# fabrii4/AutoEncoder-FFT

Measured on AMD Instinct MI355X. Metric: frames/s fwd+bwd (FFT mode, 512x512, 4 layers), higher is better.
Workload: dtype f32; 1 GPU; cfg3-P2: 512x512x3 frames, 4 pairs 3->8->16->32->64, 5x5, pool 2/layer, FFT mode, fwd + 1 loop-body iteration per pair (operator form); every step produces reconstructions, batch-mean gradients, updated weights and the per-pair post-update MSE partial sums -- the sums themselves are formed by the next step's gradient launch (no per-step MSE read-back inside the timed loop); frames_per_gpu=32, global_batch=32, parallelism=dp1

## Files before the change

### autoencoder-fft_amd/csrc/fft_kernels.hip

```cpp
#include "internal.h"
#include "device_util.h"
#include "fft_common.h"
#include <hip/hip_ext.h>
#include <math.h>
#include <map>
#include <mutex>
#include <vector>

namespace aefft {

__device__ float2 g_tw[TW_N];

hipError_t upload_twiddles(hipStream_t st)
{
    static std::vector<float2> host;
    if (host.empty()) {
        host.resize(TW_N);
        for (int k = 0; k < TW_N; ++k) {
            double a = -2.0 * M_PI * (double)k / (double)TW_N;
            host[k] = make_float2((float)cos(a), (float)sin(a));
        }
    }
    hipError_t e = hipMemcpyToSymbolAsync(HIP_SYMBOL(g_tw), host.data(), sizeof(float2) * TW_N, 0, hipMemcpyHostToDevice, st);
    if (e != hipSuccess) return e;
    return hipStreamSynchronize(st);
}

const float2* twiddle_table()
{
    void* p = nullptr;
    if (hipGetSymbolAddress(&p, HIP_SYMBOL(g_tw)) != hipSuccess) return nullptr;
    return static_cast<const float2*>(p);
}

bool fft_size_supported(int n) { return n >= 8 && n <= 2048 && (n & (n - 1)) == 0; }

template <int DIR> __device__ __forceinline__ float2 twid(int idx)
{
    float2 w = g_tw[idx];
    if (DIR > 0) w.y = -w.y;
    return w;
}

template <int N> __device__ __forceinline__ void pass_sync()
{
    if constexpr (N / 8 <= 64) __builtin_amdgcn_wave_barrier();
    else __syncthreads();
}

template <int N, int R, int S, int DIR>
__device__ __forceinline__ void fft_pass(float2* s, int t, float2 w1)
{
    constexpr int T = N / 8;
    constexpr int E = 8 / R;
    constexpr int n = N / S;
    float2 a[8];
#pragma unroll
    for (int v = 0; v < E; ++v) {
        const int ib = t + T * v;
#pragma unroll
        for (int tt = 0; tt < R; ++tt) a[v * R + tt] = s[pad_idx(ib + tt * (N / R))];
    }
    pass_sync<N>();
#pragma unroll
    for (int v = 0; v < E; ++v) {
        const int ib = t + T * v;
        const int p = ib / S, q = ib % S;
        Dft<R, DIR>::run(&a[v * R]);
        if constexpr (n > R) {
            static_assert(R == 8 && E == 1, "twiddled passes are radix 8");
            const float2 w2 = cmul(w1, w1), w3 = cmul(w2, w1), w4 = cmul(w2, w2);
            const float2 w5 = cmul(w4, w1), w6 = cmul(w3, w3), w7 = cmul(w4, w3);
            a[1] = cmul(a[1], w1); a[2] = cmul(a[2], w2); a[3] = cmul(a[3], w3); a[4] = cmul(a[4], w4);
            a[5] = cmul(a[5], w5); a[6] = cmul(a[6], w6); a[7] = cmul(a[7], w7);
        }
#pragma unroll
        for (int u = 0; u < R; ++u) s[pad_idx(q + S * (R * p + u))] = a[v * R + u];
    }
    if constexpr (S * R == N) __syncthreads();
    else pass_sync<N>();
}

template <int N, int DIR> struct FftTw {
    float2 w[3];
    __device__ __forceinline__ void load(int t)
    {
        constexpr int S[3] = {1, 8, 64};
#pragma unroll
        for (int i = 0; i < 3; ++i) {
            w[i] = make_float2(1.f, 0.f);
            if (N / S[i] > 8) {
                float2 v = g_tw[((t / S[i]) * S[i]) * (TW_N / N)];
                if (DIR > 0) v.y = -v.y;
                w[i] = v;
            }
        }
    }
};

template <int N, int S, int I, int DIR> struct Passes {
    static __device__ __forceinline__ void run(float2* s, int t, const FftTw<N, DIR>& tw)
    {
        constexpr int n = N / S;
        constexpr int R = n >= 8 ? 8 : n;
        fft_pass<N, R, S, DIR>(s, t, tw.w[I < 3 ? I : 2]);
        Passes<N, S * R, I + 1, DIR>::run(s, t, tw);
    }
};
template <int N, int I, int DIR> struct Passes<N, N, I, DIR> {
    static __device__ __forceinline__ void run(float2*, int, const FftTw<N, DIR>&) {}
};

template <int N, int DIR> __device__ __forceinline__ void fft_lds(float2* s, int t, const FftTw<N, DIR>& tw) { Passes<N, 1, 0, DIR>::run(s, t, tw); }

template <int N> struct RowCfg {
    static constexpr int T = N / 8;
    static constexpr int NT = T > 256 ? T : 256;
    static constexpr int G = NT / T;
    static constexpr int PL = pad_len(N);
};

template <int N, bool U8>
__global__ __launch_bounds__(RowCfg<N>::NT) void r2c_rows_kernel(const void* __restrict__ in_v, float2* __restrict__ mid,
                                                                   long npairs, int Wc)
{
    using Cfg = RowCfg<N>;
    constexpr int T = Cfg::T, NT = Cfg::NT, G = Cfg::G, PL = Cfg::PL;
    extern __shared__ float2 s[];
    const int tid = threadIdx.x;
    const int g = tid / T, t = tid % T;
    const long pair0 = (long)blockIdx.x * G;
    FftTw<N, -1> tws;
    tws.load(t);

    constexpr int NPOS = G * (N / 4) / NT;
    static_assert((G * (N / 4)) % NT == 0, "tile must be a whole number of positions per thread");
    const int live = npairs - pair0 < G ? (int)(npairs - pair0) : G;
    float4 va[NPOS], vb[NPOS];
    if constexpr (U8) {
        const unsigned* src = reinterpret_cast<const unsigned*>(static_cast<const unsigned char*>(in_v) + pair0 * 2 * N);
        unsigned wa[NPOS], wb[NPOS];
#pragma unroll
        for (int q = 0; q < NPOS; ++q) {
            const int pos = tid + q * NT;
            const int gg = pos / (N / 4), c4 = pos % (N / 4);
            const int idx = gg < live ? gg * (2 * N / 4) + c4 : c4;
            wa[q] = __builtin_nontemporal_load(&src[idx]);
            wb[q] = __builtin_nontemporal_load(&src[idx + N / 4]);
        }
#pragma unroll
        for (int q = 0; q < NPOS; ++q) {
            va[q] = make_float4((float)(wa[q] & 255u), (float)((wa[q] >> 8) & 255u), (float)((wa[q] >> 16) & 255u), (float)(wa[q] >> 24));
            vb[q] = make_float4((float)(wb[q] & 255u), (float)((wb[q] >> 8) & 255u), (float)((wb[q] >> 16) & 255u), (float)(wb[q] >> 24));
        }
    } else {
        const float4* src = reinterpret_cast<const float4*>(static_cast<const float*>(in_v) + pair0 * 2 * N);
#pragma unroll
        for (int q = 0; q < NPOS; ++q) {
            const int pos = tid + q * NT;
            const int gg = pos / (N / 4), c4 = pos % (N / 4);
            const int idx = gg < live ? gg * (2 * N / 4) + c4 : c4;
            va[q] = ld_stream(&src[idx]);
            vb[q] = ld_stream(&src[idx + N / 4]);
        }
    }
#pragma unroll
    for (int q = 0; q < NPOS; ++q) {
        const int pos = tid + q * NT;
        const int gg = pos / (N / 4), c4 = pos % (N / 4);
        if (gg < live) {
            float2* z = s + gg * PL + pad_idx(4 * c4);
            z[0] = make_float2(va[q].x, vb[q].x); z[1] = make_float2(va[q].y, vb[q].y);
            z[2] = make_float2(va[q].z, vb[q].z); z[3] = make_float2(va[q].w, vb[q].w);
        }
    }
    __syncthreads();
    fft_lds<N, -1>(s + g * PL, t, tws);

    const int half = Wc / 2, hs = 31 - __builtin_clz(half);
    float2* const obase = mid + pair0 * 2 * Wc;
    for (int it = tid; it < G * half; it += NT) {
        const int gg = it >> hs, k = (it & (half - 1)) * 2;
        if (gg >= live) continue;
        const float2* z = s + gg * PL;
        const float2 zk1 = z[pad_idx(k + 1)], zn1 = z[pad_idx(N - k - 1)];
        float2 a0, b0;
        if (k == 0) {
            const float2 z0 = z[pad_idx(0)], zh = z[pad_idx(N / 2)];
            a0 = make_float2(z0.x, zh.x); b0 = make_float2(z0.y, zh.y);
        } else {
            const float2 zk = z[pad_idx(k)], zn = z[pad_idx(N - k)];
            a0 = make_float2(0.5f * (zk.x + zn.x), 0.5f * (zk.y - zn.y)); b0 = make_float2(0.5f * (zk.y + zn.y), -0.5f * (zk.x - zn.x));
        }
        const float2 a1 = make_float2(0.5f * (zk1.x + zn1.x), 0.5f * (zk1.y - zn1.y)), b1 = make_float2(0.5f * (zk1.y + zn1.y), -0.5f * (zk1.x - zn1.x));
        float2* dst = obase + (gg * 2 * Wc + k);
        *reinterpret_cast<float4*>(dst) = make_float4(a0.x, a0.y, a1.x, a1.y);
        *reinterpret_cast<float4*>(dst + Wc) = make_float4(b0.x, b0.y, b1.x, b1.y);
    }
}

template <int N, bool SPARSE, bool U8 = false>
__global__ __launch_bounds__(RowCfg<N>::NT) void c2r_rows_kernel(const float2* __restrict__ mid, void* __restrict__ out_v,
                                                                   long npairs, int Wc, float scale)
{
    using Cfg = RowCfg<N>;
    constexpr int T = Cfg::T, NT = Cfg::NT, G = Cfg::G, PL = Cfg::PL;
    extern __shared__ float2 s[];
    const int tid = threadIdx.x;
    const int g = tid / T, t = tid % T;
    FftTw<N, +1> tws;
    tws.load(t);
    const long pair0 = (long)blockIdx.x * G;
    if constexpr (SPARSE) {
        static_assert(N >= 128, "sparse head: three radix-8 passes or more");
        const int live = npairs - pair0 < G ? (int)(npairs - pair0) : G;
        const float2* const ibase = mid + pair0 * 2 * Wc;
        const bool lo = t < Wc, hi = t > T - Wc;
        const int k = lo ? t : (hi ? T - t : 0);
        const bool ok = g < live && (lo || hi);
        const int off = ok ? g * 2 * Wc + k : 0;
        float2 A = ibase[off], B = ibase[off + Wc];
        if (!ok) { A = make_float2(0.f, 0.f); B = A; }
        const float2 zz = make_float2(0.f, 0.f);
        const float2 a0 = lo ? (t == 0 ? make_float2(A.x, B.x) : make_float2(A.x - B.y, A.y + B.x)) : zz;
        const float2 a4 = t == 0 ? make_float2(A.y, B.y) : zz;
        const float2 a7 = hi ? make_float2(A.x + B.y, -A.y + B.x) : zz;
        const float c = 0.70710678118654752440f;
        const float2 e = cadd(a0, a4), o = csub(a0, a4);
        const float2 r1 = make_float2(c * (a7.x + a7.y), c * (a7.y - a7.x));
        const float2 r2 = make_float2(a7.y, -a7.x);
        const float2 r3 = make_float2(c * (a7.y - a7.x), -c * (a7.x + a7.y));
        float2 x[8] = {cadd(e, a7), cadd(o, r1), cadd(e, r2), cadd(o, r3), csub(e, a7), csub(o, r1), csub(e, r2), csub(o, r3)};
        const float2 w1 = tws.w[0];
        const float2 w2 = cmul(w1, w1), w3 = cmul(w2, w1), w4 = cmul(w2, w2);
        const float2 w5 = cmul(w4, w1), w6 = cmul(w3, w3), w7 = cmul(w4, w3);
        x[1] = cmul(x[1], w1); x[2] = cmul(x[2], w2); x[3] = cmul(x[3], w3); x[4] = cmul(x[4], w4);
        x[5] = cmul(x[5], w5); x[6] = cmul(x[6], w6); x[7] = cmul(x[7], w7);
        float2* z = s + g * PL;
#pragma unroll
        for (int u = 0; u < 8; ++u) z[pad_idx(8 * t + u)] = x[u];
        pass_sync<N>();
        Passes<N, 8, 1, +1>::run(z, t, tws);
    } else {
    constexpr int NIT = G * (N / 4) / NT;
    static_assert((G * (N / 4)) % NT == 0, "tile must be a whole number of items per thread");
    float4 av[NIT], bv[NIT];
    const int live = npairs - pair0 < G ? (int)(npairs - pair0) : G;
    const float2* const ibase = mid + pair0 * 2 * Wc;
#pragma unroll
    for (int q = 0; q < NIT; ++q) {
        const int it = tid + q * NT;
        const int gg = it / (N / 4), k = (it % (N / 4)) * 2;
        const bool ok = gg < live && k < Wc;
        const int off = ok ? gg * 2 * Wc + k : 0;
        av[q] = ld_stream(reinterpret_cast<const float4*>(ibase + off));
        bv[q] = ld_stream(reinterpret_cast<const float4*>(ibase + off + Wc));
        if (!ok) { av[q] = make_float4(0.f, 0.f, 0.f, 0.f); bv[q] = av[q]; }
    }
#pragma unroll
    for (int q = 0; q < NIT; ++q) {
        const int it = tid + q * NT;
        const int gg = it / (N / 4), k = (it % (N / 4)) * 2;
        if (gg >= live) continue;
        float2* z = s + gg * PL;
        const float4 a = av[q], b = bv[q];
        if (k == 0) {
            z[pad_idx(0)] = make_float2(a.x, b.x);
            z[pad_idx(N / 2)] = make_float2(a.y, b.y);
        } else {
            z[pad_idx(k)] = make_float2(a.x - b.y, a.y + b.x);
            z[pad_idx(N - k)] = make_float2(a.x + b.y, -a.y + b.x);
        }
        z[pad_idx(k + 1)] = make_float2(a.z - b.w, a.w + b.z);
        z[pad_idx(N - k - 1)] = make_float2(a.z + b.w, -a.w + b.z);
    }
    __syncthreads();
    fft_lds<N, +1>(s + g * PL, t, tws);
    }

    constexpr int NQ = G * (N / 4) / NT;
    const int live = npairs - pair0 < G ? (int)(npairs - pair0) : G;
    if constexpr (U8) {
        unsigned* const orow = reinterpret_cast<unsigned*>(static_cast<unsigned char*>(out_v) + pair0 * 2 * N);
#pragma unroll
        for (int q = 0; q < NQ; ++q) {
            const int idx = tid + q * NT;
            const int gg = idx / (N / 4), n4 = idx % (N / 4);
            if (gg < live) {
                const float2* z = s + gg * PL + pad_idx(4 * n4);
                const float2 z0 = z[0], z1 = z[1], z2 = z[2], z3 = z[3];
                const unsigned wa = px_u8(z0.x * scale) | px_u8(z1.x * scale) << 8 | px_u8(z2.x * scale) << 16 | px_u8(z3.x * scale) << 24;
                const unsigned wb = px_u8(z0.y * scale) | px_u8(z1.y * scale) << 8 | px_u8(z2.y * scale) << 16 | px_u8(z3.y * scale) << 24;
                __builtin_nontemporal_store(wa, &orow[(gg * 2) * (N / 4) + n4]);
                __builtin_nontemporal_store(wb, &orow[(gg * 2 + 1) * (N / 4) + n4]);
            }
        }
        return;
    }
    float* const orow = static_cast<float*>(out_v) + pair0 * 2 * N;
#pragma unroll
    for (int q = 0; q < NQ; ++q) {
        const int idx = tid + q * NT;
        const int gg = idx / (N / 4), n = (idx % (N / 4)) * 4;
        if (gg < live) {
            const float2* z = s + gg * PL + pad_idx(n);
            const float2 z0 = z[0], z1 = z[1], z2 = z[2], z3 = z[3];
            st_stream(reinterpret_cast<float4*>(orow + (gg * 2) * N + n), make_float4(z0.x * scale, z1.x * scale, z2.x * scale, z3.x * scale));
            st_stream(reinterpret_cast<float4*>(orow + (gg * 2 + 1) * N + n), make_float4(z0.y * scale, z1.y * scale, z2.y * scale, z3.y * scale));
        }
    }
}

template <int N, int CW>
__global__ __launch_bounds__(CW* N / 8) void fwd_cols_kernel(const float2* __restrict__ mid, float2* __restrict__ out,
                                                              int Wc, int Nxs)
{
    constexpr int T = N / 8, NT = CW * T, PL = pad_len(N);
    extern __shared__ float2 s[];
    const int tid = threadIdx.x;
    FftTw<N, -1> tws;
    tws.load(tid % T);
    const long plane = blockIdx.x;
    const int c0 = blockIdx.y * CW;

    const float2* src = mid + plane * N * (long)Wc + c0;
    constexpr int NLD = N * (CW / 2) / NT;
    float4 val[NLD];
#pragma unroll
    for (int k = 0; k < NLD; ++k) {
        const int it = tid + k * NT;
        const float4* ptr = reinterpret_cast<const float4*>(src + ((it / (CW / 2)) * Wc + 2 * (it % (CW / 2))));
        if constexpr (CW * sizeof(float2) >= 128) val[k] = ld_stream(ptr);
        else val[k] = *ptr;
    }
#pragma unroll
    for (int k = 0; k < NLD; ++k) {
        const int it = tid + k * NT;
        const int r = it / (CW / 2), c2 = it % (CW / 2);
        s[(2 * c2) * PL + pad_idx(r)] = make_float2(val[k].x, val[k].y);
        s[(2 * c2 + 1) * PL + pad_idx(r)] = make_float2(val[k].z, val[k].w);
    }
    __syncthreads();
    fft_lds<N, -1>(s + (tid / T) * PL, tid % T, tws);

    const int Nyrs = Wc + 1;
    float2* dst = out + plane * Nxs * (long)Nyrs;
    for (int it = tid; it < Nxs * CW; it += NT) {
        const int i = it / CW, c = it % CW;
        const int si = crop_row(i, N, Nxs);
        const float2 z = s[c * PL + pad_idx(si)];
        const int col = c0 + c;
        if (col == 0) {
            const float2 zn = s[pad_idx((N - si) % N)];
            dst[i * Nyrs] = make_float2(0.5f * (z.x + zn.x), 0.5f * (z.y - zn.y));
            dst[i * Nyrs + Wc] = make_float2(0.5f * (z.y + zn.y), -0.5f * (z.x - zn.x));
        } else {
            dst[i * Nyrs + col] = z;
        }
    }
}

template <int N, int CW>
__global__ __launch_bounds__(CW* N / 8) void inv_cols_kernel(const float2* __restrict__ in, float2* __restrict__ mid,
                                                              int Wc, int Nxi, const OpIn op)
{
    constexpr int T = N / 8, NT = CW * T, PL = pad_len(N);
    extern __shared__ float2 s[];
    const int tid = threadIdx.x;
    FftTw<N, +1> tws;
    tws.load(tid % T);
    const long plane = blockIdx.x;
    const int c0 = blockIdx.y * CW;
    const int Nyri = Wc + 1;
    const float2* src = in + plane * Nxi * (long)Nyri;
    auto ld = [&](long t) { return op.A ? opin_load(op, plane, (int)t, Nxi, 2 * Wc) : src[t]; };

    float2* dcs = s + CW * PL;
    float2* nys = dcs + Nxi;
    if (Nxi < N) {
        for (int it = tid; it < CW * PL; it += NT) s[it] = make_float2(0.f, 0.f);
        __syncthreads();
    }
    constexpr int NLD = 8;
    float2 v[NLD], w[NLD];
    const int nsrc = Nxi * CW;
#pragma unroll
    for (int k = 0; k < NLD; ++k) {
        if (k * NT < nsrc) {
            const int it = min(tid + k * NT, nsrc - 1);
            const int sr = it / CW, c = it % CW;
            v[k] = ld((long)sr * Nyri + c0 + c);
            w[k] = (c0 + c == 0) ? ld((long)sr * Nyri + Wc) : make_float2(0.f, 0.f);
        }
    }
#pragma unroll
    for (int k = 0; k < NLD; ++k) {
        const int it = tid + k * NT;
        if (it < nsrc) {
            const int sr = it / CW, c = it % CW;
            if (c0 + c == 0) { dcs[sr] = v[k]; nys[sr] = w[k]; }
            else {
                const int r = Nxi == N ? sr : (sr < Nxi / 2 ? sr : (sr == Nxi / 2 ? N / 2 : sr + N - Nxi));
                s[c * PL + pad_idx(r)] = v[k];
            }
        }
    }
    if (c0 == 0) {
        __syncthreads();
        for (int r = tid; r < N; r += NT) {
            const int sr = padsrc_row(r, N, Nxi), sm = padsrc_row((N - r) % N, N, Nxi);
            const float2 zz = make_float2(0.f, 0.f);
            const float2 d0 = sr >= 0 ? dcs[sr] : zz, n0 = sr >= 0 ? nys[sr] : zz, d1 = sm >= 0 ? dcs[sm] : zz, n1 = sm >= 0 ? nys[sm] : zz;
            const float2 dc = make_float2(0.5f * (d0.x + d1.x), 0.5f * (d0.y - d1.y));
            const float2 ny = make_float2(0.5f * (n0.x + n1.x), 0.5f * (n0.y - n1.y));
            s[pad_idx(r)] = make_float2(dc.x - ny.y, dc.y + ny.x);
        }
    }
    __syncthreads();
    fft_lds<N, +1>(s + (tid / T) * PL, tid % T, tws);

    float2* dst = mid + plane * N * (long)Wc + c0;
    for (int it = tid; it < N * (CW / 2); it += NT) {
        const int r = it / (CW / 2), c2 = it % (CW / 2);
        const float2 a = s[(2 * c2) * PL + pad_idx(r)], b = s[(2 * c2 + 1) * PL + pad_idx(r)];
        *reinterpret_cast<float4*>(dst + (long)r * Wc + 2 * c2) = make_float4(a.x, a.y, b.x, b.y);
    }
}

template <int M> struct BluCfg {
    static constexpr int T = M / 8;
    static constexpr int NT = T > 256 ? T : 256;
    static constexpr int G = NT / T;
    static constexpr int PL = pad_len(M);
};

template <int M, int MODE>
__global__ __launch_bounds__(BluCfg<M>::NT) void bluestein_rows_kernel(const void* __restrict__ in_, void* __restrict__ out_, const float2* __restrict__ tab,
                                                                        long nrows, int n, float scale)
{
    using Cfg = BluCfg<M>;
    constexpr int T = Cfg::T, NT = Cfg::NT, G = Cfg::G, PL = Cfg::PL;
    extern __shared__ float2 s[];
    const int tid = threadIdx.x, g = tid / T, t = tid % T;
    const long row = (long)blockIdx.x * G + g;
    const bool live = row < nrows;
    FftTw<M, -1> twf;
    FftTw<M, +1> twi;
    twf.load(t); twi.load(t);
    float2* z = s + g * PL;
    const float2* const bhat = tab;
    const float2* const w = tab + M;
    const int nh = n / 2 + 1;
    for (int j = t; j < M; j += T) {
        float2 v = make_float2(0.f, 0.f);
        if (live && j < n) {
            if (MODE == 0) v = reinterpret_cast<const float2*>(in_)[row * n + j];
            else if (MODE == 1) v = make_float2(reinterpret_cast<const float*>(in_)[row * n + j], 0.f);
            else {
                const float2* X = reinterpret_cast<const float2*>(in_) + row * nh;
                if (j < nh) { v = X[j]; if (j == 0 || 2 * j == n) v.y = 0.f; }
                else { v = X[n - j]; v.y = -v.y; }
            }
            v = cmul(v, w[j]);
        }
        z[pad_idx(j)] = v;
    }
    __syncthreads();
    fft_lds<M, -1>(z, t, twf);
    for (int j = t; j < M; j += T) z[pad_idx(j)] = cmul(z[pad_idx(j)], bhat[j]);
    __syncthreads();
    fft_lds<M, +1>(z, t, twi);
    if (!live) return;
    const float sc = scale / (float)M;
    const int nout = MODE == 1 ? nh : n;
    for (int k = t; k < nout; k += T) {
        float2 v = cmul(z[pad_idx(k)], w[k]);
        if (MODE == 2) reinterpret_cast<float*>(out_)[row * n + k] = v.x * sc;
        else reinterpret_cast<float2*>(out_)[row * nout + k] = make_float2(v.x * sc, v.y * sc);
    }
}

__global__ __launch_bounds__(256) void transpose_c_kernel(const float2* __restrict__ in, float2* __restrict__ out, int R, int C)
{
    __shared__ float2 tile[32][33];
    const long plane = blockIdx.z;
    const int r0 = blockIdx.y * 32, c0 = blockIdx.x * 32;
    const int tx = threadIdx.x % 32, ty = threadIdx.x / 32;
    for (int k = ty; k < 32; k += 8) if (r0 + k < R && c0 + tx < C) tile[k][tx] = in[(plane * R + r0 + k) * C + c0 + tx];
    __syncthreads();
    for (int k = ty; k < 32; k += 8) if (c0 + k < C && r0 + tx < R) out[(plane * C + c0 + k) * R + r0 + tx] = tile[tx][k];
}

size_t fft_mid_elems(long planes, int Nx, int Wc) { return (size_t)planes * Nx * Wc; }

template <typename K> static hipError_t allow_lds(K kernel, size_t bytes)
{
    if (bytes <= 64 * 1024) return hipSuccess;
    return hipFuncSetAttribute(reinterpret_cast<const void*>(kernel), hipFuncAttributeMaxDynamicSharedMemorySize, (int)bytes);
}

template <int N> static hipError_t run_r2c_rows(const void* in, float2* mid, long npairs, int Wc, hipStream_t st, bool in_u8)
{
    using Cfg = RowCfg<N>;
    const size_t lds = sizeof(float2) * (Cfg::G * Cfg::PL);
    hipError_t e = in_u8 ? allow_lds(r2c_rows_kernel<N, true>, lds) : allow_lds(r2c_rows_kernel<N, false>, lds);
    if (e != hipSuccess) return e;
    const long blocks = (npairs + Cfg::G - 1) / Cfg::G;
    if (in_u8) r2c_rows_kernel<N, true><<<dim3((unsigned)blocks), dim3(Cfg::NT), lds, st>>>(in, mid, npairs, Wc);
    else r2c_rows_kernel<N, false><<<dim3((unsigned)blocks), dim3(Cfg::NT), lds, st>>>(in, mid, npairs, Wc);
    return hipGetLastError();
}
template <int N, bool SPARSE, bool U8> static hipError_t run_c2r_rows_as(const float2* mid, void* out, long npairs, int Wc, float scale, hipStream_t st)
{
    using Cfg = RowCfg<N>;
    const size_t lds = sizeof(float2) * (Cfg::G * Cfg::PL);
    const long blocks = (npairs + Cfg::G - 1) / Cfg::G;
    hipError_t e = allow_lds(c2r_rows_kernel<N, SPARSE, U8>, lds);
    if (e != hipSuccess) return e;
    c2r_rows_kernel<N, SPARSE, U8><<<dim3((unsigned)blocks), dim3(Cfg::NT), lds, st>>>(mid, out, npairs, Wc, scale);
    return hipGetLastError();
}
template <int N> static hipError_t run_c2r_rows(const float2* mid, void* out, long npairs, int Wc, float scale, hipStream_t st, bool out_u8)
{
    if constexpr (N >= 128) {
        if (Wc <= N / 16)
            return out_u8 ? run_c2r_rows_as<N, true, true>(mid, out, npairs, Wc, scale, st) : run_c2r_rows_as<N, true, false>(mid, out, npairs, Wc, scale, st);
    }
    return out_u8 ? run_c2r_rows_as<N, false, true>(mid, out, npairs, Wc, scale, st) : run_c2r_rows_as<N, false, false>(mid, out, npairs, Wc, scale, st);
}
template <int N, int CW> static hipError_t run_fwd_cols(const float2* mid, float2* out, long planes, int Wc, int Nxs, hipStream_t st, hipEvent_t done)
{
    const size_t lds = sizeof(float2) * (CW * pad_len(N));
    hipError_t e = allow_lds(fwd_cols_kernel<N, CW>, lds);
    if (e != hipSuccess) return e;
    if (done) hipExtLaunchKernelGGL((fwd_cols_kernel<N, CW>), dim3((unsigned)planes, Wc / CW), dim3(CW * N / 8), lds, st, nullptr, done, 0, mid, out, Wc, Nxs);
    else fwd_cols_kernel<N, CW><<<dim3((unsigned)planes, Wc / CW), dim3(CW * N / 8), lds, st>>>(mid, out, Wc, Nxs);
    return hipGetLastError();
}
static OpIn g_opin_none{};
template <int N, int CW> static hipError_t run_inv_cols(const float2* in, float2* mid, long planes, int Wc, int Nxi, hipStream_t st, const OpIn& op = g_opin_none)
{
    const size_t lds = sizeof(float2) * (CW * pad_len(N) + 2 * Nxi);
    hipError_t e = allow_lds(inv_cols_kernel<N, CW>, lds);
    if (e != hipSuccess) return e;
    inv_cols_kernel<N, CW><<<dim3((unsigned)planes, Wc / CW), dim3(CW * N / 8), lds, st>>>(in, mid, Wc, Nxi, op);
    return hipGetLastError();
}

template <int N, bool FWD> static hipError_t cols_dispatch(const float2* a, float2* b, long planes, int Wc, int Nother, hipStream_t st, const OpIn& op = g_opin_none, hipEvent_t done = nullptr)
{
    constexpr int CWMAX = (8192 / N) < 16 ? (8192 / N) : 16;
    int cw = CWMAX;
    while (cw > Wc) cw >>= 1;
    if (!FWD) while (cw > 4 && planes * (Wc / cw) < 256) cw >>= 1;
#define AEFFT_CW_CASE(C)                                                                                   \
    if constexpr (C <= CWMAX) {                                                                             \
        if (cw == C) return FWD ? run_fwd_cols<N, C>(a, b, planes, Wc, Nother, st, done) : run_inv_cols<N, C>(a, b, planes, Wc, Nother, st, op); \
    }
    AEFFT_CW_CASE(16) AEFFT_CW_CASE(8) AEFFT_CW_CASE(4)
#undef AEFFT_CW_CASE
    return hipErrorInvalidValue;
}

#define AEFFT_N_SWITCH(n, CALL)                       \
    switch (n) {                                      \
    case 8: { constexpr int NN = 8; CALL; }           \
    case 16: { constexpr int NN = 16; CALL; }         \
    case 32: { constexpr int NN = 32; CALL; }         \
    case 64: { constexpr int NN = 64; CALL; }         \
    case 128: { constexpr int NN = 128; CALL; }       \
    case 256: { constexpr int NN = 256; CALL; }       \
    case 512: { constexpr int NN = 512; CALL; }       \
    case 1024: { constexpr int NN = 1024; CALL; }     \
    case 2048: { constexpr int NN = 2048; CALL; }     \
    default: e = hipErrorInvalidValue;                \
    }

bool fft_size_supported_any(int n) { return fft_size_supported(n) || (n >= 8 && n <= 1024 && (n & 1) == 0); }
static int blu_m(int n) { int m = 16; while (m < 2 * n - 1) m *= 2; return m; }
struct BluKey { int dev, n, dir; bool operator<(const BluKey& o) const { return dev != o.dev ? dev < o.dev : (n != o.n ? n < o.n : dir < o.dir); } };
#define AEFFT_M_SWITCH(m, CALL)                      \
    switch (m) {                                      \
    case 16: { constexpr int MM = 16; CALL; }         \
    case 32: { constexpr int MM = 32; CALL; }         \
    case 64: { constexpr int MM = 64; CALL; }         \
    case 128: { constexpr int MM = 128; CALL; }       \
    case 256: { constexpr int MM = 256; CALL; }       \
    case 512: { constexpr int MM = 512; CALL; }       \
    case 1024: { constexpr int MM = 1024; CALL; }     \
    case 2048: { constexpr int MM = 2048; CALL; }     \
    default: e = hipErrorInvalidValue;                \
    }
static std::mutex g_blu_mu;
static std::vector<float2> blu_host_table(int n, int dir)
{
    const int M = blu_m(n);
    std::vector<double> wr(n), wi(n), cr(M), ci(M);
    for (int j = 0; j < n; ++j) {
        const long q = ((long)j * j) % (2L * n);
        wr[j] = cos(M_PI * (double)q / n); wi[j] = dir * sin(M_PI * (double)q / n);
    }
    for (int m = 0; m < M; ++m) { cr[m] = cos(2.0 * M_PI * m / M); ci[m] = -sin(2.0 * M_PI * m / M); }
    std::vector<float2> t(M + n);
    for (int k = 0; k < M; ++k) {
        double ar = 0.0, ai = 0.0;
        for (int j = 0; j < M; ++j) {
            const int jj = j < n ? j : (M - j < n ? M - j : -1);
            if (jj < 0) continue;
            const double br = wr[jj], bi = -wi[jj];
            const int m = (int)(((long)j * k) % M);
            ar += br * cr[m] - bi * ci[m]; ai += br * ci[m] + bi * cr[m];
        }
        t[k] = make_float2((float)ar, (float)ai);
    }
    for (int j = 0; j < n; ++j) t[M + j] = make_float2((float)wr[j], (float)wi[j]);
    return t;
}
static hipError_t blu_table(int n, int dir, const float2** out)
{
    static std::map<BluKey, float2*> cache;
    int dev = 0;
    hipError_t e = hipGetDevice(&dev);
    if (e != hipSuccess) return e;
    const BluKey key{dev, n, dir};
    std::lock_guard<std::mutex> lock(g_blu_mu);
    auto it = cache.find(key);
    if (it == cache.end()) {
        const std::vector<float2> host = blu_host_table(n, dir);
        float2* p = nullptr;
        e = hipMalloc(&p, sizeof(float2) * host.size());
        if (e != hipSuccess) return e;
        e = hipMemcpy(p, host.data(), sizeof(float2) * host.size(), hipMemcpyHostToDevice);
        if (e != hipSuccess) { (void)hipFree(p); return e; }
        it = cache.emplace(key, p).first;
    }
    *out = it->second;
    return hipSuccess;
}
template <int M, int MODE> static hipError_t run_blu_rows(const void* in, void* out, const float2* tab, long nrows, int n, float scale, hipStream_t st)
{
    using Cfg = BluCfg<M>;
    const size_t lds = sizeof(float2) * (size_t)Cfg::G * Cfg::PL;
    hipError_t e = allow_lds(bluestein_rows_kernel<M, MODE>, lds);
    if (e != hipSuccess) return e;
    const long blocks = (nrows + Cfg::G - 1) / Cfg::G;
    if (blocks >= (1L << 31)) return hipErrorInvalidValue;
    bluestein_rows_kernel<M, MODE><<<dim3((unsigned)blocks), dim3(Cfg::NT), lds, st>>>(in, out, tab, nrows, n, scale);
    return hipGetLastError();
}
static hipError_t blu_rows(int mode, const void* in, void* out, long nrows, int n, int dir, float scale, hipStream_t st)
{
    const float2* tab = nullptr;
    hipError_t e = blu_table(n, dir, &tab);
    if (e != hipSuccess) return e;
    const int M = blu_m(n);
    if (mode == 0) { AEFFT_M_SWITCH(M, e = (run_blu_rows<MM, 0>(in, out, tab, nrows, n, scale, st)); break) }
    else if (mode == 1) { AEFFT_M_SWITCH(M, e = (run_blu_rows<MM, 1>(in, out, tab, nrows, n, scale, st)); break) }
    else { AEFFT_M_SWITCH(M, e = (run_blu_rows<MM, 2>(in, out, tab, nrows, n, scale, st)); break) }
    return e;
}
static hipError_t transpose_c(const float2* in, float2* out, long planes, int R, int C, hipStream_t st)
{
    constexpr long ZMAX = 65535;
    for (long p0 = 0; p0 < planes; p0 += ZMAX) {
        const long np = planes - p0 < ZMAX ? planes - p0 : ZMAX;
        const long off = p0 * R * (long)C;
        transpose_c_kernel<<<dim3((C + 31) / 32, (R + 31) / 32, (unsigned)np), 256, 0, st>>>(in + off, out + off, R, C);
        hipError_t e = hipGetLastError();
        if (e != hipSuccess) return e;
    }
    return hipSuccess;
}
size_t fft_any_ws_elems(long planes, int Nx, int Ny) { return (size_t)planes * Nx * (Ny / 2 + 1); }
hipError_t launch_r2c_any(const float* in, float2* out, float2* w1, float2* w2, long planes, int Nx, int Ny, hipStream_t st)
{
    if (!fft_size_supported_any(Nx) || !fft_size_supported_any(Ny) || Nx > 1024 || Ny > 1024) return hipErrorInvalidValue;
    if (planes <= 0) return hipSuccess;
    const int Nyr = Ny / 2 + 1;
    hipError_t e = blu_rows(1, in, w1, planes * Nx, Ny, -1, 1.f, st);
    if (e == hipSuccess) e = transpose_c(w1, w2, planes, Nx, Nyr, st);
    if (e == hipSuccess) e = blu_rows(0, w2, w1, planes * Nyr, Nx, -1, 1.f, st);
    if (e == hipSuccess) e = transpose_c(w1, out, planes, Nyr, Nx, st);
    return e;
}
hipError_t launch_c2r_any(const float2* in, float* out, float2* w1, float2* w2, long planes, int Nx, int Ny, float scale, hipStream_t st)
{
    if (!fft_size_supported_any(Nx) || !fft_size_supported_any(Ny) || Nx > 1024 || Ny > 1024) return hipErrorInvalidValue;
    if (planes <= 0) return hipSuccess;
    const int Nyr = Ny / 2 + 1;
    hipError_t e = transpose_c(in, w1, planes, Nx, Nyr, st);
    if (e == hipSuccess) e = blu_rows(0, w1, w2, planes * Nyr, Nx, +1, 1.f, st);
    if (e == hipSuccess) e = transpose_c(w2, w1, planes, Nyr, Nx, st);
    if (e == hipSuccess) e = blu_rows(2, w1, out, planes * Nx, Ny, +1, scale, st);
    return e;
}

static bool rows_pow2(int Ny, int Wc) { return fft_size_supported(Ny) && Wc >= 4 && (Wc & (Wc - 1)) == 0; }
static bool cols_pow2(int Nx, int Wc) { return fft_size_supported(Nx) && Wc >= 4 && ((Wc & (Wc - 1)) == 0 || Wc % 16 == 0); }
static bool axis_ok(int n) { return fft_size_supported(n) || fft_size_mixed(n); }

hipError_t launch_r2c(const void* in, float2* out, float2* mid, long planes, int Nx, int Ny, int Nxs, int Nys, hipStream_t st, hipEvent_t done, bool in_u8)
{
    if (!fft_size_supported(Nx) || !fft_size_supported(Ny) || Nxs > Nx || Nys > Ny || Nys < 8 || Nxs < 2 || (Nys & (Nys - 1)) || (Nxs & 1)) {
        if (!axis_ok(Nx) || !axis_ok(Ny) || Nxs > Nx || Nys > Ny || Nxs < 2 || Nys < 2 || (Nxs & 1) || (Nys & 1)) return hipErrorInvalidValue;
        if (planes <= 0) return hipSuccess;
        const int Wc = Nys / 2;
        const long npairs = planes * Nx / 2;
        hipError_t e = hipSuccess;
        if (in) {
            if (rows_pow2(Ny, Wc)) { AEFFT_N_SWITCH(Ny, e = run_r2c_rows<NN>(in, mid, npairs, Wc, st, in_u8); break) }
            else e = launch_mix_r2c_rows(in, mid, npairs, Ny, Wc, st, in_u8);
            if (e != hipSuccess) return e;
        }
        if (out) {
            if (cols_pow2(Nx, Wc)) { AEFFT_N_SWITCH(Nx, e = (cols_dispatch<NN, true>(mid, out, planes, Wc, Nxs, st, g_opin_none, done)); break) }
            else e = launch_mix_fwd_cols(mid, out, planes, Nx, Wc, Nxs, st, done);
        }
        return e;
    }
    if (planes <= 0) return hipSuccess;
    const int Wc = Nys / 2;
    const long npairs = planes * Nx / 2;
    hipError_t e = hipSuccess;
    if (in) {
        AEFFT_N_SWITCH(Ny, e = run_r2c_rows<NN>(in, mid, npairs, Wc, st, in_u8); break)
        if (e != hipSuccess) return e;
    }
    if (out) {
        AEFFT_N_SWITCH(Nx, e = (cols_dispatch<NN, true>(mid, out, planes, Wc, Nxs, st, g_opin_none, done)); break)
    }
    return e;
}

hipError_t launch_c2r(const float2* in, void* out, float2* mid, long planes, int Nxi, int Nyi, int Nx, int Ny, float scale, hipStream_t st, const OpIn* opin,
                      bool out_u8)
{
    const OpIn op = opin ? *opin : g_opin_none;
    if ((Nxi == Nx) != (Nyi == Ny)) return hipErrorInvalidValue;
    if (!fft_size_supported(Nx) || !fft_size_supported(Ny) || Nxi > Nx || Nyi > Ny || Nyi < 8 || Nxi < 2 || (Nyi & 1) || (Nxi & 1)) {
        if (!axis_ok(Nx) || !axis_ok(Ny) || Nxi > Nx || Nyi > Ny || Nxi < 2 || Nyi < 2 || (Nxi & 1) || (Nyi & 1)) return hipErrorInvalidValue;
        if (planes <= 0) return hipSuccess;
        const int Wc = Nyi / 2;
        const long npairs = planes * Nx / 2;
        hipError_t e = hipSuccess;
        if (in || op.A) {
            if (cols_pow2(Nx, Wc)) { AEFFT_N_SWITCH(Nx, e = (cols_dispatch<NN, false>(in, mid, planes, Wc, Nxi, st, op)); break) }
            else e = launch_mix_inv_cols(in, mid, planes, Nx, Wc, Nxi, st, op.A ? &op : nullptr);
            if (e != hipSuccess) return e;
        }
        if (out) {
            if (rows_pow2(Ny, Wc)) { AEFFT_N_SWITCH(Ny, e = run_c2r_rows<NN>(mid, out, npairs, Wc, scale, st, out_u8); break) }
            else e = launch_mix_c2r_rows(mid, out, npairs, Ny, Wc, scale, st, out_u8);
        }
        return e;
    }
    if (planes <= 0) return hipSuccess;
    const int Wc = Nyi / 2;
    const long npairs = planes * Nx / 2;
    hipError_t e = hipSuccess;
    if (in || op.A) {
        AEFFT_N_SWITCH(Nx, e = (cols_dispatch<NN, false>(in, mid, planes, Wc, Nxi, st, op)); break)
        if (e != hipSuccess) return e;
    }
    if (out) {
        AEFFT_N_SWITCH(Ny, e = run_c2r_rows<NN>(mid, out, npairs, Wc, scale, st, out_u8); break)
    }
    return e;
}

}
```

Before: 221,800 frames/s.

## Use two-pass radix-16x32 FFT with permlane16 exchange for N=512

Adds a dedicated 512-point FFT plan in which 32 threads each run a radix-16 DFT. A permlane16 swap handles part of the second stage, so there are two LDS passes instead of three radix-8 passes. Row and column kernels for N=512 now use 32 threads per transform and 128-thread row blocks, and the sparse c2r head is rewritten for this shape. The aim is fewer LDS round-trips and barriers, at the cost of more registers per thread (16 complex values), which may lower occupancy.

Result: no change. 222,200 frames/s (median of 4 runs) (+0.2%).

```diff
diff --git a/autoencoder-fft_amd/csrc/fft_kernels.hip b/autoencoder-fft_amd/csrc/fft_kernels.hip
--- a/autoencoder-fft_amd/csrc/fft_kernels.hip
+++ b/autoencoder-fft_amd/csrc/fft_kernels.hip
@@ -113,9 +113,109 @@
 
 template <int N, int DIR> __device__ __forceinline__ void fft_lds(float2* s, int t, const FftTw<N, DIR>& tw) { Passes<N, 1, 0, DIR>::run(s, t, tw); }
 
+template <int N> struct FftShape {
+    static constexpr bool TWO = N == 512;
+    static constexpr int T = TWO ? 32 : N / 8;
+};
+
+template <int DIR> struct Dft<16, DIR> {
+    static __device__ __forceinline__ void run(float2* a)
+    {
+        float2 e[8] = {a[0], a[2], a[4], a[6], a[8], a[10], a[12], a[14]};
+        float2 o[8] = {a[1], a[3], a[5], a[7], a[9], a[11], a[13], a[15]};
+        Dft<8, DIR>::run(e);
+        Dft<8, DIR>::run(o);
+        const float c = 0.70710678118654752440f, c1 = 0.92387953251128675613f, s1 = 0.38268343236508977173f;
+        const float2 cc = make_float2(c, c), nc = make_float2(-c, -c);
+        const float2 o1 = cmul(o[1], make_float2(c1, DIR * s1)), o3 = cmul(o[3], make_float2(s1, DIR * c1));
+        const float2 o5 = cmul(o[5], make_float2(-s1, DIR * c1)), o7 = cmul(o[7], make_float2(-c1, DIR * s1));
+        const float2 o2 = cc * add_muli<DIR>(o[2], o[2]);
+        const float2 o6 = nc * sub_muli<DIR>(o[6], o[6]);
+        a[0] = cadd(e[0], o[0]); a[8] = csub(e[0], o[0]);
+        a[1] = cadd(e[1], o1);   a[9] = csub(e[1], o1);
+        a[2] = cadd(e[2], o2);   a[10] = csub(e[2], o2);
+        a[3] = cadd(e[3], o3);   a[11] = csub(e[3], o3);
+        a[4] = add_muli<DIR>(e[4], o[4]); a[12] = sub_muli<DIR>(e[4], o[4]);
+        a[5] = cadd(e[5], o5);   a[13] = csub(e[5], o5);
+        a[6] = cadd(e[6], o6);   a[14] = csub(e[6], o6);
+        a[7] = cadd(e[7], o7);   a[15] = csub(e[7], o7);
+    }
+};
+
+template <int DIR> struct FftTw512 {
+    float2 v1, v8, t16;
+    __device__ __forceinline__ void load(int t)
+    {
+        v1 = twid<DIR>(t * (TW_N / 512));
+        v8 = twid<DIR>(8 * t * (TW_N / 512));
+        t16 = twid<DIR>((t & 15) * (TW_N / 32));
+    }
+};
+
+__device__ __forceinline__ void lane16_swap(float2& a, float2& b)
+{
+    const auto x = __builtin_amdgcn_permlane16_swap(__float_as_uint(a.x), __float_as_uint(b.x), false, false);
+    const auto y = __builtin_amdgcn_permlane16_swap(__float_as_uint(a.y), __float_as_uint(b.y), false, false);
+    a = make_float2(__uint_as_float(x[0]), __uint_as_float(y[0]));
+    b = make_float2(__uint_as_float(x[1]), __uint_as_float(y[1]));
+}
+
+template <int DIR> __device__ __forceinline__ void fft512_exchange(float2* s, int t, const FftTw512<DIR>& tw, float2* a)
+{
+    const float2 v1 = tw.v1, v8 = tw.v8;
+    const float2 v2 = cmul(v1, v1), v3 = cmul(v2, v1), v4 = cmul(v2, v2);
+    const float2 v5 = cmul(v4, v1), v6 = cmul(v3, v3), v7 = cmul(v4, v3);
+    a[1] = cmul(a[1], v1); a[2] = cmul(a[2], v2); a[3] = cmul(a[3], v3); a[4] = cmul(a[4], v4);
+    a[5] = cmul(a[5], v5); a[6] = cmul(a[6], v6); a[7] = cmul(a[7], v7); a[8] = cmul(a[8], v8);
+    a[9] = cmul(a[9], cmul(v8, v1)); a[10] = cmul(a[10], cmul(v8, v2)); a[11] = cmul(a[11], cmul(v8, v3)); a[12] = cmul(a[12], cmul(v8, v4));
+    a[13] = cmul(a[13], cmul(v8, v5)); a[14] = cmul(a[14], cmul(v8, v6)); a[15] = cmul(a[15], cmul(v8, v7));
+    float2* z = s + 34 * (t & 15) + (t >> 4);
+#pragma unroll
+    for (int j = 0; j < 8; ++j) {
+        lane16_swap(a[2 * j], a[2 * j + 1]);
+        z[2 * j] = cadd(a[2 * j], a[2 * j + 1]);
+        z[2 * j + 16] = cmul(csub(a[2 * j], a[2 * j + 1]), tw.t16);
+    }
+    __builtin_amdgcn_wave_barrier();
+}
+
+template <int DIR> __device__ __forceinline__ void fft512_pass2(float2* s, int t)
+{
+    float2 a[16];
+#pragma unroll
+    for (int b = 0; b < 16; ++b) a[b] = s[34 * b + t];
+    __builtin_amdgcn_wave_barrier();
+    Dft<16, DIR>::run(a);
+    float2* z = s + pad_idx(t);
+#pragma unroll
+    for (int u = 0; u < 16; ++u) z[pad_idx(32 * u)] = a[u];
+    __syncthreads();
+}
+
+template <int DIR> __device__ __forceinline__ void fft512_lds(float2* s, int t, const FftTw512<DIR>& tw)
+{
+    float2 a[16];
+    const float2* z = s + pad_idx(t);
+#pragma unroll
+    for (int m = 0; m < 16; ++m) a[m] = z[pad_idx(32 * m)];
+    __builtin_amdgcn_wave_barrier();
+    Dft<16, DIR>::run(a);
+    fft512_exchange<DIR>(s, t, tw, a);
+    fft512_pass2<DIR>(s, t);
+}
+
+template <int N, int DIR> struct FftPlan {
+    using Tw = FftTw<N, DIR>;
+    static __device__ __forceinline__ void run(float2* s, int t, const Tw& tw) { fft_lds<N, DIR>(s, t, tw); }
+};
+template <int DIR> struct FftPlan<512, DIR> {
+    using Tw = FftTw512<DIR>;
+    static __device__ __forceinline__ void run(float2* s, int t, const Tw& tw) { fft512_lds<DIR>(s, t, tw); }
+};
+
 template <int N> struct RowCfg {
-    static constexpr int T = N / 8;
-    static constexpr int NT = T > 256 ? T : 256;
+    static constexpr int T = FftShape<N>::T;
+    static constexpr int NT = FftShape<N>::TWO ? 128 : (T > 256 ? T : 256);
     static constexpr int G = NT / T;
     static constexpr int PL = pad_len(N);
 };
@@ -130,7 +230,7 @@
     const int tid = threadIdx.x;
     const int g = tid / T, t = tid % T;
     const long pair0 = (long)blockIdx.x * G;
-    FftTw<N, -1> tws;
+    typename FftPlan<N, -1>::Tw tws;
     tws.load(t);
 
     constexpr int NPOS = G * (N / 4) / NT;
@@ -175,7 +275,7 @@
         }
     }
     __syncthreads();
-    fft_lds<N, -1>(s + g * PL, t, tws);
+    FftPlan<N, -1>::run(s + g * PL, t, tws);
 
     const int half = Wc / 2, hs = 31 - __builtin_clz(half);
     float2* const obase = mid + pair0 * 2 * Wc;
@@ -208,10 +308,31 @@
     extern __shared__ float2 s[];
     const int tid = threadIdx.x;
     const int g = tid / T, t = tid % T;
-    FftTw<N, +1> tws;
+    typename FftPlan<N, +1>::Tw tws;
     tws.load(t);
     const long pair0 = (long)blockIdx.x * G;
-    if constexpr (SPARSE) {
+    if constexpr (SPARSE && FftShape<N>::TWO) {
+        const int live = npairs - pair0 < G ? (int)(npairs - pair0) : G;
+        const float2* const ibase = mid + pair0 * 2 * Wc;
+        const bool lo = g < live && t < Wc, hi = g < live && t > T - Wc;
+        const int offl = lo ? g * 2 * Wc + t : 0, offh = hi ? g * 2 * Wc + (T - t) : 0;
+        float2 A = ibase[offl], B = ibase[offl + Wc], C = ibase[offh], D = ibase[offh + Wc];
+        const float2 zz = make_float2(0.f, 0.f);
+        const float2 a0 = lo ? (t == 0 ? make_float2(A.x, B.x) : make_float2(A.x - B.y, A.y + B.x)) : zz;
+        const float2 a8 = lo && t == 0 ? make_float2(A.y, B.y) : zz;
+        const float2 aF = hi ? make_float2(C.x + D.y, -C.y + D.x) : zz;
+        const float c = 0.70710678118654752440f, c1 = 0.92387953251128675613f, s1 = 0.38268343236508977173f;
+        const float2 e = cadd(a0, a8), o = csub(a0, a8);
+        const float2 r[8] = {aF, cmul(aF, make_float2(c1, -s1)), make_float2(c * (aF.x + aF.y), c * (aF.y - aF.x)), cmul(aF, make_float2(s1, -c1)),
+                             make_float2(aF.y, -aF.x), cmul(aF, make_float2(-s1, -c1)), make_float2(c * (aF.y - aF.x), -c * (aF.x + aF.y)),
+                             cmul(aF, make_float2(-c1, -s1))};
+        float2 x[16];
+#pragma unroll
+        for (int k = 0; k < 8; ++k) { x[k] = cadd(k & 1 ? o : e, r[k]); x[k + 8] = csub(k & 1 ? o : e, r[k]); }
+        float2* z = s + g * PL;
+        fft512_exchange<+1>(z, t, tws, x);
+        fft512_pass2<+1>(z, t);
+    } else if constexpr (SPARSE) {
         static_assert(N >= 128, "sparse head: three radix-8 passes or more");
         const int live = npairs - pair0 < G ? (int)(npairs - pair0) : G;
         const float2* const ibase = mid + pair0 * 2 * Wc;
@@ -275,7 +396,7 @@
         z[pad_idx(N - k - 1)] = make_float2(a.z + b.w, -a.w + b.z);
     }
     __syncthreads();
-    fft_lds<N, +1>(s + g * PL, t, tws);
+    FftPlan<N, +1>::run(s + g * PL, t, tws);
     }
 
     constexpr int NQ = G * (N / 4) / NT;
@@ -312,13 +433,13 @@
 }
 
 template <int N, int CW>
-__global__ __launch_bounds__(CW* N / 8) void fwd_cols_kernel(const float2* __restrict__ mid, float2* __restrict__ out,
+__global__ __launch_bounds__(CW* FftShape<N>::T) void fwd_cols_kernel(const float2* __restrict__ mid, float2* __restrict__ out,
                                                               int Wc, int Nxs)
 {
-    constexpr int T = N / 8, NT = CW * T, PL = pad_len(N);
+    constexpr int T = FftShape<N>::T, NT = CW * T, PL = pad_len(N);
     extern __shared__ float2 s[];
     const int tid = threadIdx.x;
-    FftTw<N, -1> tws;
+    typename FftPlan<N, -1>::Tw tws;
     tws.load(tid % T);
     const long plane = blockIdx.x;
     const int c0 = blockIdx.y * CW;
@@ -341,7 +462,7 @@
         s[(2 * c2 + 1) * PL + pad_idx(r)] = make_float2(val[k].z, val[k].w);
     }
     __syncthreads();
-    fft_lds<N, -1>(s + (tid / T) * PL, tid % T, tws);
+    FftPlan<N, -1>::run(s + (tid / T) * PL, tid % T, tws);
 
     const int Nyrs = Wc + 1;
     float2* dst = out + plane * Nxs * (long)Nyrs;
@@ -361,13 +482,13 @@
 }
 
 template <int N, int CW>
-__global__ __launch_bounds__(CW* N / 8) void inv_cols_kernel(const float2* __restrict__ in, float2* __restrict__ mid,
+__global__ __launch_bounds__(CW* FftShape<N>::T) void inv_cols_kernel(const float2* __restrict__ in, float2* __restrict__ mid,
                                                               int Wc, int Nxi, const OpIn op)
 {
-    constexpr int T = N / 8, NT = CW * T, PL = pad_len(N);
+    constexpr int T = FftShape<N>::T, NT = CW * T, PL = pad_len(N);
     extern __shared__ float2 s[];
     const int tid = threadIdx.x;
-    FftTw<N, +1> tws;
+    typename FftPlan<N, +1>::Tw tws;
     tws.load(tid % T);
     const long plane = blockIdx.x;
     const int c0 = blockIdx.y * CW;
@@ -381,7 +502,7 @@
         for (int it = tid; it < CW * PL; it += NT) s[it] = make_float2(0.f, 0.f);
         __syncthreads();
     }
-    constexpr int NLD = 8;
+    constexpr int NLD = N / T;
     float2 v[NLD], w[NLD];
     const int nsrc = Nxi * CW;
 #pragma unroll
@@ -417,7 +538,7 @@
         }
     }
     __syncthreads();
-    fft_lds<N, +1>(s + (tid / T) * PL, tid % T, tws);
+    FftPlan<N, +1>::run(s + (tid / T) * PL, tid % T, tws);
 
     float2* dst = mid + plane * N * (long)Wc + c0;
     for (int it = tid; it < N * (CW / 2); it += NT) {
@@ -533,8 +654,8 @@
     const size_t lds = sizeof(float2) * (CW * pad_len(N));
     hipError_t e = allow_lds(fwd_cols_kernel<N, CW>, lds);
     if (e != hipSuccess) return e;
-    if (done) hipExtLaunchKernelGGL((fwd_cols_kernel<N, CW>), dim3((unsigned)planes, Wc / CW), dim3(CW * N / 8), lds, st, nullptr, done, 0, mid, out, Wc, Nxs);
-    else fwd_cols_kernel<N, CW><<<dim3((unsigned)planes, Wc / CW), dim3(CW * N / 8), lds, st>>>(mid, out, Wc, Nxs);
+    if (done) hipExtLaunchKernelGGL((fwd_cols_kernel<N, CW>), dim3((unsigned)planes, Wc / CW), dim3(CW * FftShape<N>::T), lds, st, nullptr, done, 0, mid, out, Wc, Nxs);
+    else fwd_cols_kernel<N, CW><<<dim3((unsigned)planes, Wc / CW), dim3(CW * FftShape<N>::T), lds, st>>>(mid, out, Wc, Nxs);
     return hipGetLastError();
 }
 static OpIn g_opin_none{};
@@ -543,7 +664,7 @@
     const size_t lds = sizeof(float2) * (CW * pad_len(N) + 2 * Nxi);
     hipError_t e = allow_lds(inv_cols_kernel<N, CW>, lds);
     if (e != hipSuccess) return e;
-    inv_cols_kernel<N, CW><<<dim3((unsigned)planes, Wc / CW), dim3(CW * N / 8), lds, st>>>(in, mid, Wc, Nxi, op);
+    inv_cols_kernel<N, CW><<<dim3((unsigned)planes, Wc / CW), dim3(CW * FftShape<N>::T), lds, st>>>(in, mid, Wc, Nxi, op);
     return hipGetLastError();
 }
 
```
